# dohlee/diffab-pytorch

Measured on AMD Instinct MI355X. Metric: CDR-residue denoise-steps/sec (K=128 patch), higher is better.
Workload: dtype f32 (bf16x6 / fp16x3 split-precision products on the 16-bit matrix cores, fp32 accumulate; fp32-accurate, DESIGN section 4)

## Files before the change

### diffab-pytorch_amd/csrc/api.hip

```cpp
#include <atomic>
#include <cstring>
#include <mutex>
#include <vector>

#include "common.h"
#include "denoiser_internal.h"
#include "mlp_chain_tile.h"
#include "../../include/diffab_hip_debug.h"

namespace diffab {

static thread_local char g_err[512] = "";

void set_error(const char* fmt, ...) {
  va_list ap;
  va_start(ap, fmt);
  vsnprintf(g_err, sizeof(g_err), fmt, ap);
  va_end(ap);
}

namespace {
struct OrderState {
  std::recursive_mutex mu;
  hipStream_t last = nullptr;
// ... 362 lines not shown
  int* row_plan;
  unsigned char* start_class;
  float* beta_traj;
  int* ctx_of_row;
  float* res_ctx;
  void* step;
  size_t bytes;
};

static SampleBuffers carve_sample(const diffab_dims* d, void* ws, int n_pair = 0, bool mapped = false) {
  Carver c(ws);
  const size_t rows = static_cast<size_t>(d->B) * d->K;
  SampleBuffers s;
  s.beta = c.take<float>(d->B);
  s.eps = c.take<float>(rows * 3);
  s.O0 = c.take<float>(rows * 9);
  s.post = c.take<float>(rows * d->V);
  s.t_dev = c.take<int>(64);
  s.tiles = c.take<unsigned char>(static_cast<size_t>(d->B) * ((d->K + 15) / 16));
  s.row_plan = c.take<int>(static_cast<size_t>(d->B) * (2 + (d->K + 15) / 16));
  s.beta_traj = c.take<float>(static_cast<size_t>(3) * kTrajRows * d->D);
  s.ctx_of_row = mapped ? c.take<int>(d->B) : nullptr;
  s.res_ctx = mapped ? c.take<float>(rows * d->D) : nullptr;
  const size_t step_bytes = carve_step(d, nullptr, n_pair).bytes;
  s.step = c.take<char>(step_bytes);
  s.start_class = c.take<unsigned char>((static_cast<size_t>(d->B) + 3) & ~static_cast<size_t>(3));
  s.bytes = c.bytes();
  return s;
}

struct ScoreBuffers {
  int* t_list;
  float* beta;
  int* ctx_of_row;
  int64_t* seq_t;
  float *x_t, *O_t, *eps, *eps_hat;
  float* res_ctx;
  void* step;
  size_t bytes;
};
static ScoreBuffers carve_score(const diffab_dims* d, void* ws, int n_ctx) {
  Carver c(ws);
  const size_t rows = static_cast<size_t>(d->B) * d->K;
  ScoreBuffers s;
  s.t_list = c.take<int>(kTrajRows);
  s.beta = c.take<float>(d->B);
  s.ctx_of_row = c.take<int>(d->B);
  s.seq_t = c.take<int64_t>(rows);
  s.x_t = c.take<float>(rows * 3);
  s.O_t = c.take<float>(rows * 9);
  s.eps = c.take<float>(rows * 3);
  s.eps_hat = c.take<float>(rows * 3);
  s.res_ctx = c.take<float>(rows * d->D);
  s.step = c.take<char>(carve_step(d, nullptr, n_ctx).bytes);
  s.bytes = c.bytes();
  return s;
}

}

using namespace diffab;

extern "C" {

const char* diffab_version(void) { return "diffab_hip 0.1.0 (gfx950)"; }
const char* diffab_last_error(void) { return g_err; }

int diffab_device_ok(void) {
  int n = 0;
  if (hipGetDeviceCount(&n) != hipSuccess || n <= 0) return 0;
  hipDeviceProp_t p;
  int dev = 0;
  if (hipGetDevice(&dev) != hipSuccess || hipGetDeviceProperties(&p, dev) != hipSuccess) return 0;
  return std::strncmp(p.gcnArchName, "gfx950", 6) == 0 ? 1 : 0;
}

int diffab_debug_linear128(const float* X, const float* W, const float* bias, float* Y, int64_t M, int32_t Kd, int32_t mode, void* scratch,
                           size_t scratch_bytes, void* stream) {
  StreamOrder order_(stream);
  DIFFAB_REQUIRE(X && W && Y && M >= 1 && M < (1LL << 31) && Kd >= 32 && Kd % 32 == 0, DIFFAB_ERR_ARG, "debug_linear128: bad operands");
  hipStream_t st = as_stream(stream);
  if (mode == 0) return launch_linear(X, Kd, W, bias, Y, 128, static_cast<int>(M), 128, Kd, false, st);
  if (int rc = require_aligned16("debug_linear128", {{"X", X}, {"W", W}, {"bias", bias}, {"Y", Y}})) return rc;
  if (mode == 2) {
    const size_t pb = (rowgemm128_h3_planes_bytes(Kd) + 255) & ~static_cast<size_t>(255);
    DIFFAB_REQUIRE(Kd % 64 == 0, DIFFAB_ERR_ARG, "debug_linear128: mode 2 (fp16 x 3) needs Kd %% 64 == 0 (its chunks of 32 k are joined in pairs)");
    DIFFAB_REQUIRE(scratch && scratch_bytes >= pb + 512 && rowgemm128_b6_ok(X, Kd, Y, 128, static_cast<int>(M), Kd) &&
                       (reinterpret_cast<uintptr_t>(scratch) & 15) == 0,
                   DIFFAB_ERR_ARG, "debug_linear128: mode 2 needs 16-byte aligned operands and %zu bytes of scratch", pb + 512);
    float* wis = reinterpret_cast<float*>(static_cast<char*>(scratch) + pb);
    if (int rc = launch_wsplit128_h3(W, Kd, Kd, scratch, wis, st)) return rc;
    return launch_rowgemm128_h3p(X, Kd, scratch, wis, bias, nullptr, 0, Y, 128, static_cast<int>(M), Kd, false, st, nullptr);
  }
  DIFFAB_REQUIRE(mode == 1 && scratch && scratch_bytes >= rowgemm128_b6_scratch_bytes(Kd) && rowgemm128_b6_ok(X, Kd, Y, 128, static_cast<int>(M), Kd),
                 DIFFAB_ERR_ARG, "debug_linear128: mode 1 needs 16-byte aligned operands and %zu bytes of scratch", rowgemm128_b6_scratch_bytes(Kd));
  return launch_rowgemm128_b6(X, Kd, W, Kd, bias, nullptr, 0, Y, 128, static_cast<int>(M), Kd, false, scratch, st);
}

int diffab_debug_xstat128(const float* X, const float* W, float* Y, int64_t M, int32_t N, int32_t mode, void* scratch, size_t scratch_bytes,
                          void* stream) {
  StreamOrder order_(stream);
  DIFFAB_REQUIRE(X && W && Y && scratch && M >= 1 && M < (1LL << 31) && N >= 1 && (mode == 1 || mode == 2), DIFFAB_ERR_ARG,
                 "debug_xstat128: bad operands");
  const size_t need = mode == 1 ? xstat_b6_scratch_bytes(N) : xstat_h3_scratch_bytes(N);
  if (int rc = require_aligned16("debug_xstat128", {{"X", X}, {"W", W}, {"Y", Y}})) return rc;
  DIFFAB_REQUIRE(scratch_bytes >= need && (reinterpret_cast<uintptr_t>(scratch) & 15) == 0 && (reinterpret_cast<uintptr_t>(X) & 15) == 0,
                 DIFFAB_ERR_ARG, "debug_xstat128: needs 16-byte aligned X / scratch and %zu bytes of scratch", need);
  hipStream_t st = as_stream(stream);
  if (mode == 1) return launch_xstat_b6(X, W, 1, N, Y, N, static_cast<int>(M), N, scratch, st);
  return launch_xstat_h3(X, W, 1, N, Y, N, static_cast<int>(M), N, scratch, st);
}

int diffab_debug_dense_forms(int64_t rows, int32_t nblocks, int32_t has_parts, int32_t* out5) {
  DIFFAB_REQUIRE(out5 && rows >= 1 && rows < (1LL << 31) && nblocks >= 1, DIFFAB_ERR_ARG, "debug_dense_forms: bad operands");
  const int M = static_cast<int>(rows);
  const int group = rowgemm128_rows_per_group(M, has_parts != 0);
  out5[0] = group;
  out5[1] = M % (group == 0 ? 64 : group) != 0;
  out5[2] = dense_tile_full(M);
  out5[3] = dense_tile_nsplit(M, nblocks);
  out5[4] = M - (M - 1) / kDenseTileRows * kDenseTileRows;
  return DIFFAB_OK;
}

int diffab_debug_gemm_tn(const float* A, const float* B, float* C, float* db, int64_t M, int32_t N1, int32_t N2, int32_t mode, void* stream) {
  StreamOrder order_(stream);
  DIFFAB_REQUIRE(A && B && C && M >= 1 && M < (1LL << 31) && N1 >= 1 && N2 >= 1 && (mode == 1 || mode == 2), DIFFAB_ERR_ARG,
                 "debug_gemm_tn: bad operands");
  hipStream_t st = as_stream(stream);
  if (mode == 1) return launch_gemm_tn_b6(A, N1, B, N2, C, N2, static_cast<int>(M), N1, N2, db, nullptr, nullptr, 0, st);
  return launch_gemm_tn_h3(A, N1, B, N2, C, N2, static_cast<int>(M), N1, N2, db, nullptr, nullptr, 0, st);
}

int diffab_set_stream_guard(int on) {
  set_stream_order(on != 0);
  return DIFFAB_OK;
}

int diffab_debug_set_module_stagger(int32_t ticks_10ns, int32_t classes) {
  set_module_stagger(ticks_10ns, classes);
  return DIFFAB_OK;
}

int diffab_debug_set_module_stamps(void* device_buffer) {
  set_module_stamps(device_buffer);
  return DIFFAB_OK;
}

int diffab_debug_row_tiles(const uint8_t* gen_mask, int32_t B, int32_t K, uint8_t* tiles, void* stream) {
  StreamOrder order_(stream);
  DIFFAB_REQUIRE(gen_mask && tiles && B >= 1 && K >= 16 && K % 16 == 0, DIFFAB_ERR_ARG, "debug_row_tiles: need B >= 1 and K a multiple of 16");
  return launch_tiles_needed(gen_mask, B, K, tiles, as_stream(stream));
}

int diffab_debug_row_plan(const uint8_t* gen_mask, int32_t B, int32_t K, int32_t* plan, void* stream) {
  StreamOrder order_(stream);
  DIFFAB_REQUIRE(gen_mask && plan && B >= 1 && K >= 16 && K <= 1024 && K % 16 == 0, DIFFAB_ERR_ARG,
                 "debug_row_plan: need B >= 1 and K a multiple of 16 in 16 .. 1024");
  return launch_row_plan(gen_mask, B, K, plan, as_stream(stream));
}

int diffab_debug_start_classes(const int32_t* plan, int32_t B, int32_t K, int32_t classes, uint8_t* out, int32_t on_device, void* stream) {
  DIFFAB_REQUIRE(plan && out && B >= 1 && K >= 16 && K <= 1024 && K % 16 == 0 && classes >= 1 && classes <= 256, DIFFAB_ERR_ARG,
                 "debug_start_classes: need B >= 1, K a multiple of 16 in 16 .. 1024 and 1 .. 256 classes");
  if (on_device) {
    StreamOrder order_(stream);
    return launch_start_classes(plan, B, K, classes, out, as_stream(stream));
  }
  for (int b = 0; b < B; ++b) out[b] = static_cast<uint8_t>(start_class_of(plan, B, K, classes, b));
  return DIFFAB_OK;
}

int diffab_debug_set_attn_variant(int32_t v) { return set_attn_variant(v); }

// ... 674 lines not shown
```

### diffab-pytorch_amd/csrc/denoiser_internal.h

```cpp
#pragma once
#include "common.h"

namespace diffab {

int launch_linear_generic(const float* X, int ldx, const float* W, const float* bias, float* Y, int ldy, int M, int N, int Kd, bool relu,
                          hipStream_t st);
size_t ipa_generic_workspace_floats(const diffab_dims* d);
int ipa_layer_generic(const diffab_dims* d, const diffab_ipa_layer_weights* w, const float* x, const float* e, const float* R, const float* t,
                      float* y, float* ws, hipStream_t st, const int* ctx_of_row = nullptr);
int launch_embed_concat(const float* res_ctx, const float* emb, const int64_t* seq, int D, int64_t rows, float* out, hipStream_t st);
int launch_beta_concat(const float* h, const float* beta, int D, int K, int64_t rows, float* out, hipStream_t st);
int launch_heads_finish(const float* v, const float* O_t, const float* logits, int V, int64_t rows, float* O0, float* post, hipStream_t st);
int launch_proj_frames_f32(const float* x, const float* const* W6, const float* R, const float* t, float* proj, int rows, hipStream_t st);
int launch_losses_bwd(const float* post, const float* tpost, const float* eps, const float* teps, const float* O0, const float* tO,
                      const float* O_t, const float* v, const uint8_t* gm, const uint8_t* rm, const float* count, const float* up, int V,
                      int64_t rows, float* d_logits, float* d_eps, float* d_v, hipStream_t st);
int launch_heads_cotangent(const float* post, const float* c_post, const float* c_eps, const float* c_O0, const float* O_t, const float* v,
                           int V, int64_t rows, float* d_logits, float* d_eps, float* d_v, float* d_Ot, hipStream_t st);
int launch_ipa_frames_bwd(const float* proj, const float* dproj, int NP, int pt_col0, int n_pts, const float* feat, const float* dfeat, int F,
                          int ol_col0, int on_col0, int n_vpts, const float* R, const float* t, float* dR, float* dt, int rows,
                          hipStream_t st);

constexpr int kDenseTileRows = 128;
constexpr int kDenseFillGroups = 256;
constexpr int kPartsTilesMax = 64;
inline int rowgemm128_rows_per_group(int M, bool parts_usable) {
  if (parts_usable && (M + 63) / 64 <= kPartsTilesMax) return 0;
  return (M + kDenseTileRows - 1) / kDenseTileRows >= kDenseFillGroups ? 128 : 64;
}
inline bool dense_tile_full(int rows) { return rows % kDenseTileRows == 0; }
inline int dense_tile_nsplit(int rows, int nblocks) {
  const int ntiles = (rows + kDenseTileRows - 1) / kDenseTileRows, nsplit = kDenseFillGroups / ntiles;
  return nsplit < 1 ? 1 : (nsplit > nblocks ? nblocks : nsplit);
}

bool fast_path_supported(const diffab_dims* d);
size_t ipa_fast_workspace_floats(const diffab_dims* d);
int ipa_layer_fast(const diffab_dims* d, const diffab_ipa_layer_weights* w, const float* x, const float* e, const float* R, const float* t,
                   float* y, float* ws, hipStream_t st,
                   float* sp_keep = nullptr, float* d2_keep = nullptr,
                   const void* planes = nullptr,
                   const float* pair_planes = nullptr,
                   bool fp32_gemm = false,
                   bool taped = false,
                   const unsigned char* tile_needed = nullptr,
                   const int* ctx_of_row = nullptr, int n_ctx = 0);
bool pair_planes_supported(const diffab_dims* d);
size_t pair_planes_floats(const diffab_dims* d, int n_pair = 0);
int launch_pair_split(const diffab_dims* d, const float* e, float* planes, hipStream_t st, int n_pair = 0);
const float* pair_row_scales(const diffab_dims* d, const float* planes, int n_pair = 0);
int launch_linear(const float* X, int ldx, const float* W, const float* bias, float* Y, int ldy, int M, int N, int Kd, bool relu,
                  hipStream_t st);

bool rowgemm128_ok(const float* X, int ldx, const float* Y, int ldy, int M, int Kd);
int launch_rowgemm128(const float* X, int ldx, const float* W, int ldw, const float* bias, const int64_t* bias_idx, int bias_div, float* Y,
                      int ldy, int M, int Kd, bool relu, hipStream_t st);
size_t rowgemm128_b6_scratch_bytes(int Kd);
bool rowgemm128_b6_ok(const float* X, int ldx, const float* Y, int ldy, int M, int Kd);
int launch_wsplit128(const float* W, int ldw, int Kd, void* planes, hipStream_t st, int nrows = 128);
int launch_mlp_chains_b6(const float* X, int ldx, int nchains, const void* const* planes, const float* const* bias, const int64_t* bias_idx0,
                         int bias_div0, int nlayers, const int* n_out, float* const* Y, const int* ldy, int M, hipStream_t st);
struct MlpChainSet;
int make_mlp_chain_set(MlpChainSet* out, int nchains, const void* const* planes, const float* const* bias, const int64_t* bias_idx0,
                       int bias_div0, int nlayers, const int* n_out, float* const* Y, const int* ldy);
int launch_mlp_chain_b6(const float* X, int ldx, const void* const* planes, const float* const* bias, const int64_t* bias_idx0, int bias_div0,
                        int nlayers, int n_out, float* Y, int ldy, int M, hipStream_t st);
int launch_wsplit128_strided(const float* W, int64_t sn, int64_t sk, int kseg, int k0, void* planes, hipStream_t st);
int launch_wsplit128_segs(const float* const* W, const int* k_end, int nseg, void* planes, hipStream_t st);
int launch_rowgemm128_b6p(const float* X, int ldx, const void* planes, const float* bias, const int64_t* bias_idx, int bias_div, float* Y,
                          int ldy, int M, int Kd, bool relu, hipStream_t st, float* parts = nullptr);
size_t rowgemm128_b6_parts_floats(int M, int Kd);
size_t rowgemm128_h3_parts_floats(int M, int Kd);
int launch_rowgemm128_b6(const float* X, int ldx, const float* W, int ldw, const float* bias, const int64_t* bias_idx, int bias_div, float* Y,
                         int ldy, int M, int Kd, bool relu, void* scratch, hipStream_t st);
bool use_b6_gemm(uint32_t flags = 0);
size_t xstat_b6_scratch_bytes(int N);
int launch_gemm_tn_h3(const float* A, int lda, const float* B, int ldb, float* C, int ldc, int M, int N1, int N2, float* db,
                      float* const* seg_ptrs, const int* seg_ends, int nseg, hipStream_t st);
size_t xstat_h3_scratch_bytes(int N);
int launch_xstat_h3(const float* X, const float* W, int64_t sn, int64_t sk, float* Y, int ldy, int rows, int N, void* scratch, hipStream_t st);
int launch_xstat_b6(const float* X, const float* W, int64_t sn, int64_t sk, float* Y, int ldy, int rows, int N, void* scratch, hipStream_t st);
bool gemm_tn_b6_ok(const float* A, int lda, const float* B, int ldb, int M, int N1, int N2);
int launch_gemm_tn_b6(const float* A, int lda, const float* B, int ldb, float* C, int ldc, int M, int N1, int N2, float* db,
                      float* const* seg_ptrs, const int* seg_ends, int nseg, hipStream_t st);
size_t ipa_layer_planes_bytes();
size_t ipa_layer_small_offset();
size_t ipa_layer_h3_pj_offset();
size_t ipa_layer_h3_out_offset();
size_t ipa_layer_h3_wis_offset();
size_t rowgemm128_h3_planes_bytes(int Kd);
size_t proj_frames_h3_planes_bytes();
int launch_wsplit128_h3(const float* W, int ldw, int Kd, void* planes, float* wis, hipStream_t st, int nrows = 128);
int launch_pjsplit_h3(const float* const* W6, void* planes, float* wis, hipStream_t st);
int launch_rowgemm128_h3p(const float* X, int ldx, const void* planes, const float* wis, const float* bias, const int64_t* bias_idx, int bias_div,
                          float* Y, int ldy, int M, int Kd, bool relu, hipStream_t st, float* parts = nullptr);
int launch_proj_frames_h3p(const float* x, const void* planes, const float* wis, const float* R, const float* t, float* proj, int rows,
                           hipStream_t st);
int ipa_layer_split_weights(const diffab_ipa_layer_weights* w, void* planes, hipStream_t st);
bool ipa_module_persistent_supported(const diffab_dims* d);
int launch_ipa_module_persistent(const diffab_dims* d, float* xa, float* xb, const float* R, const float* t, float* ws, const void* planes,
                                 const float* pair_planes, hipStream_t st, const float* emb_X = nullptr, const MlpChainSet* emb = nullptr,
                                 const MlpChainSet* heads = nullptr, const int* ctx_of_row = nullptr, int n_ctx = 0,
                                 const int* last_layer_rows = nullptr,
                                 const unsigned char* start_class = nullptr);
int module_stagger_classes();
void set_module_stagger(int ticks, int classes);
void set_module_stamps(void* device_buffer);
int launch_fold_embed_table(const diffab_dims* d, const diffab_denoiser_weights* w, float* emb_tab, hipStream_t st);
int launch_fold_beta_table(const diffab_dims* d, const diffab_denoiser_weights* w, const float* beta, float* beta_tab, hipStream_t st,
                           const float* sched_beta = nullptr, int t = 0, const int* t_dev = nullptr);

bool pair_embed_fused_supported(const diffab_ctx_dims* d);
size_t pair_embed_fused_prep_floats(const diffab_ctx_dims* d);
int launch_pair_embed_fused(const diffab_ctx_dims* d, const diffab_pair_emb_weights* w, const int64_t* seq_idx, const float* distmat,
                            const float* xyz, const float* pairwise_dihedrals, const int64_t* residue_idx, int32_t residue_idx_batch_stride,
                            const int64_t* chain_idx, const float* atom_mask, const uint8_t* sequence_context_mask, float* out, float* prep,
                            float* tape_h1, float* tape_df, float* tape_m1, float* tape_m2, int64_t row0, int64_t nrows, hipStream_t st,
                            const float** coef_sp_out = nullptr);
int launch_softplus_table(const float* coefw, int n, float* out, hipStream_t st);

bool attention_split_supported(const diffab_dims* d);
size_t attention_split_workspace_floats(const diffab_dims* d);
int launch_ipa_logits(const diffab_dims* d, const float* proj, const float* gamma, float* SP, hipStream_t st);
int launch_attention_probs(const diffab_dims* d, const float* proj, const float* e, const float* Wb, const float* gamma, float* P,
                           float* D2, hipStream_t st);
constexpr int kDeLayersMax = 6;
int launch_pair_de_layers(const diffab_dims* d, int nl, const float* const* P, const float* const* G, const float* const* doe,
                          const float* const* Wb, float* de, hipStream_t st);
int launch_pair_stream_bwd(const diffab_dims* d, const float* e, const float* P, float* G , const float* D2,
                           const float* dfeat, float* wb_part, const float* Wb, float* de ,
                           hipStream_t st);
int launch_attention_split(const diffab_dims* d, const float* proj, const float* e, const float* R, const float* t, const float* Wb,
                           const float* gamma, float* feat, float* SP, hipStream_t st, float* D2 = nullptr);

void set_stream_order(bool on);
int set_attn_variant(int v);
void set_attn_stamps(void* device_buffer);

void timer_begin(hipStream_t st);
void timer_end(hipStream_t st);
bool kernel_timer_enabled();

struct Geometry {
  int rows, NP, F;
  size_t HKK;
  explicit Geometry(const diffab_dims* d)
      : rows(d->B * d->K), NP(3 * d->H * d->DS + 2 * d->H * d->PQ * 3 + d->H * d->PV * 3),
        F(d->H * d->DS + d->H * d->C + d->H * d->PV * 3 + d->H * d->PV), HKK(static_cast<size_t>(d->B) * d->H * d->K * d->K) {}
  size_t per_row(size_t n) const { return static_cast<size_t>(rows) * n; }
};

constexpr int kMaxLayers = 16;
struct BackwardPlan {
  bool fast;
  bool probs_on_tape;
  bool de_slots;
  bool split_planes;
};
BackwardPlan plan_backward(const diffab_dims* d);
struct TrainTape {
  float *cat2, *h1, *x[kMaxLayers + 1], *ipa_ws[kMaxLayers], *cat3, *t1[3], *t2[3], *vbuf, *logits;
  float* scratch;
  void* planes;
  float *sp[kMaxLayers], *d2[kMaxLayers];
  size_t floats;
};
TrainTape carve_tape(const diffab_dims* d, float* base);
inline size_t train_tape_floats(const diffab_dims* d) { return carve_tape(d, nullptr).floats; }
constexpr size_t kAttnBwdLdsMax = 160 * 1024;
size_t attn_bwd_lds_bytes(const diffab_dims* d);
inline bool attn_bwd_lds_ok(const diffab_dims* d) { return attn_bwd_lds_bytes(d) <= kAttnBwdLdsMax; }
size_t train_bwd_workspace_floats(const diffab_dims* d);
enum BwdRoot { BWD_LOSSES, BWD_COTANGENTS, BWD_LAYER };
struct BackwardArgs {
  BwdRoot root;
  const diffab_dims* d;
  const diffab_denoiser_weights *w, *g;
  TrainTape tp;
  float* ws;
  hipStream_t st;
  const int64_t* seq_t;
  const float *trans, *rot, *pair_ctx;
  const float *eps_hat, *O0_hat, *true_post, *true_eps, *true_O0, *upstream3;
  const uint8_t *gm, *rm;
  const float* post_hat;
  const float *cot_eps, *cot_O0, *cot_post;
  const float* layer_dy;
  float *layer_dx, *d_res_ctx, *d_pair_ctx, *d_trans, *d_rot;
};
int run_backward(const BackwardArgs& a);
// ... 145 lines not shown
```

### diffab-pytorch_amd/csrc/gemm_f16x3.hip

```cpp
#include "common.h"
#include "denoiser_internal.h"
#include "proj_frames_h3_tile.h"
#include "rowgemm_h3_tile.h"

namespace diffab {

using h3tile::BK;
using h3tile::h3_scale;
using h3tile::split2;

__global__ __launch_bounds__(256) void wsplit128_h3_kernel(const float* __restrict__ W, int ldw, int Kd, _Float16* __restrict__ out,
                                                          float* __restrict__ wis, int nrows) {
  const int n = blockIdx.x, tid = threadIdx.x;
  const float* row = W + static_cast<int64_t>(n) * ldw;
  float m = 0.0f;
  if (n < nrows)
    for (int k = tid; k < Kd; k += 256) m = fmaxf(m, fabsf(row[k]));
#pragma unroll
  for (int o = 1; o < 64; o <<= 1) m = fmaxf(m, __shfl_xor(m, o));
  __shared__ float wm[4];
  if ((tid & 63) == 0) wm[tid >> 6] = m;
  __syncthreads();
  m = fmaxf(fmaxf(wm[0], wm[1]), fmaxf(wm[2], wm[3]));
  float s, is;
  h3_scale(m, s, is);
  if (tid == 0) wis[n] = is;
  for (int k = tid; k < Kd; k += 256) {
    _Float16 h1, h2;
    split2(n < nrows ? row[k] * s : 0.0f, h1, h2);
    const int chunk = k / BK, kk = k % BK;
    const size_t base = (static_cast<size_t>(chunk) * 2 * 128 + n) * BK + kk;
    out[base] = h1;
    out[base + 128 * BK] = h2;
  }
}

template <bool RELU, int ROWS>
__global__ __launch_bounds__(ROWS * 4) void rowgemm128_h3_kernel(const float* __restrict__ X, int ldx, const _Float16* __restrict__ Wc,
                                                                 const float* __restrict__ wis, const float* __restrict__ bias,
                                                                 const int64_t* __restrict__ bias_idx, int bias_div, float* __restrict__ Y,
                                                                 int ldy, int M, int Kd) {
  extern __shared__ __attribute__((aligned(16))) _Float16 h3_lds[];
  h3tile::rowgemm128_h3_tile<RELU, ROWS>(h3_lds, threadIdx.x, blockIdx.x, X, ldx, Wc, wis, bias, bias_idx, bias_div, Y, ldy, M, Kd);
}
template <int ROWS>
__global__ __launch_bounds__(ROWS * 4) void rowgemm128_h3_parts_kernel(const float* __restrict__ X, int ldx, const _Float16* __restrict__ Wc, int M,
                                                                       int Kd, float* __restrict__ parts) {
  extern __shared__ __attribute__((aligned(16))) _Float16 h3_lds[];
  float* mine = parts + (static_cast<size_t>(blockIdx.x) * gridDim.y + blockIdx.y) * (ROWS * 128);
  h3tile::rowgemm128_h3_tile<false, ROWS, true>(h3_lds, threadIdx.x, blockIdx.x, X, ldx, Wc, nullptr, nullptr, nullptr, 0, nullptr, 0, M, Kd,
                                                blockIdx.y * h3tile::PART_CHUNKS, mine);
}
template <bool RELU, int ROWS>
__global__ __launch_bounds__(256) void rowgemm128_h3_parts_sum_kernel(const float* __restrict__ parts, int nparts, const float* __restrict__ wis,
                                                                      const float* __restrict__ bias, const int64_t* __restrict__ bias_idx,
                                                                      int bias_div, float* __restrict__ Y, int ldy, int M) {
  const int gid = blockIdx.x * 256 + threadIdx.x;
  const int row = gid >> 5, col = (gid & 31) * 4;
  if (row >= M) return;
  const float* src = parts + (static_cast<size_t>(row / ROWS) * nparts * ROWS + row % ROWS) * 128 + col;
  h3tile::f32x4 tot = {0.f, 0.f, 0.f, 0.f};
  for (int p = 0; p < nparts; ++p) {
    const h3tile::f32x4 v = *reinterpret_cast<const h3tile::f32x4*>(src + static_cast<size_t>(p) * (ROWS * 128));
#pragma unroll
    for (int c = 0; c < 4; ++c) tot[c] += v[c];
  }
  const bool table = bias_idx != nullptr || bias_div > 0;
  const float* brow = table ? bias + (bias_idx ? bias_idx[row] : row / bias_div) * 128 : bias;
#pragma unroll
  for (int c = 0; c < 4; ++c) {
    float o = __builtin_fmaf(tot[c], wis[col + c], brow ? brow[col + c] : 0.f);
    if (RELU) o = fmaxf(o, 0.f);
    Y[static_cast<int64_t>(row) * ldy + col + c] = o;
  }
}

size_t rowgemm128_h3_planes_bytes(int Kd) { return static_cast<size_t>(2) * 128 * Kd * sizeof(_Float16); }
bool rowgemm128_h3_ok(const float* X, int ldx, const float* Y, int ldy, int M, int Kd) {
  return Kd % BK == 0 && Kd >= BK && ldx % 4 == 0 && ldy % 4 == 0 && (reinterpret_cast<uintptr_t>(X) & 15) == 0 &&
         (reinterpret_cast<uintptr_t>(Y) & 15) == 0 && M >= 1;
}
int launch_wsplit128_h3(const float* W, int ldw, int Kd, void* planes, float* wis, hipStream_t st, int nrows) {
  DIFFAB_REQUIRE(W && planes && wis && (reinterpret_cast<uintptr_t>(planes) & 15) == 0 && Kd % BK == 0 && nrows >= 1 && nrows <= 128, DIFFAB_ERR_ARG,
                 "wsplit128_h3: bad operands");
  hipLaunchKernelGGL(wsplit128_h3_kernel, dim3(128), dim3(256), 0, st, W, ldw, Kd, static_cast<_Float16*>(planes), wis, nrows);
  DIFFAB_LAUNCH_CHECK();
  return DIFFAB_OK;
}
size_t rowgemm128_h3_parts_floats(int M, int Kd) {
  const size_t tiles64 = static_cast<size_t>((M + 63) / 64);
  return tiles64 <= kPartsTilesMax ? tiles64 * ((Kd / BK + h3tile::PART_CHUNKS - 1) / h3tile::PART_CHUNKS) * 64 * 128 : 0;
}
int launch_rowgemm128_h3p(const float* X, int ldx, const void* planes, const float* wis, const float* bias, const int64_t* bias_idx, int bias_div,
                          float* Y, int ldy, int M, int Kd, bool relu, hipStream_t st, float* parts) {
  DIFFAB_REQUIRE(rowgemm128_h3_ok(X, ldx, Y, ldy, M, Kd) && planes && wis && (reinterpret_cast<uintptr_t>(planes) & 15) == 0, DIFFAB_ERR_ARG,
                 "rowgemm128_h3: unsupported operands");
  const _Float16* Wc = static_cast<const _Float16*>(planes);
  const int tiles64 = (M + 63) / 64, nparts = (Kd / BK + h3tile::PART_CHUNKS - 1) / h3tile::PART_CHUNKS;
  const int rows_wg = rowgemm128_rows_per_group(M, parts && nparts > 1 && (reinterpret_cast<uintptr_t>(parts) & 15) == 0);
  if (rows_wg == 0) {
    DIFFAB_HIP_CHECK(hipFuncSetAttribute(reinterpret_cast<const void*>(rowgemm128_h3_parts_kernel<64>), hipFuncAttributeMaxDynamicSharedMemorySize,
                                         h3tile::lds_bytes<64>()));
    hipLaunchKernelGGL((rowgemm128_h3_parts_kernel<64>), dim3(tiles64, nparts), dim3(256), h3tile::lds_bytes<64>(), st, X, ldx, Wc, M, Kd, parts);
    const dim3 sgrid((M * 32 + 255) / 256);
    if (relu) hipLaunchKernelGGL((rowgemm128_h3_parts_sum_kernel<true, 64>), sgrid, dim3(256), 0, st, parts, nparts, wis, bias, bias_idx, bias_div, Y, ldy, M);
    else hipLaunchKernelGGL((rowgemm128_h3_parts_sum_kernel<false, 64>), sgrid, dim3(256), 0, st, parts, nparts, wis, bias, bias_idx, bias_div, Y, ldy, M);
    DIFFAB_LAUNCH_CHECK();
    return DIFFAB_OK;
  }
#define H3_LAUNCH(RELU_, ROWS_)                                                                                                          \
  do {                                                                                                                                   \
    DIFFAB_HIP_CHECK(hipFuncSetAttribute(reinterpret_cast<const void*>(rowgemm128_h3_kernel<RELU_, ROWS_>),                               \
                                         hipFuncAttributeMaxDynamicSharedMemorySize, h3tile::lds_bytes<ROWS_>()));                      \
    hipLaunchKernelGGL((rowgemm128_h3_kernel<RELU_, ROWS_>), dim3((M + ROWS_ - 1) / ROWS_), dim3(ROWS_ * 4), h3tile::lds_bytes<ROWS_>(), st, \
                       X, ldx, Wc, wis, bias, bias_idx, bias_div, Y, ldy, M, Kd);                                                        \
  } while (0)
  if (rows_wg == 128) {
    if (relu) H3_LAUNCH(true, 128);
    else H3_LAUNCH(false, 128);
  } else {
    if (relu) H3_LAUNCH(true, 64);
    else H3_LAUNCH(false, 64);
  }
#undef H3_LAUNCH
  DIFFAB_LAUNCH_CHECK();
  return DIFFAB_OK;
}

__global__ __launch_bounds__(64) void pjsplit_h3_kernel(const float* __restrict__ W0, const float* __restrict__ W1, const float* __restrict__ W2,
                                                        const float* __restrict__ W3, const float* __restrict__ W4, const float* __restrict__ W5,
                                                        _Float16* __restrict__ out, float* __restrict__ wis) {
  using namespace pjh3;
  const int gc = blockIdx.x, lane = threadIdx.x;
  const float* Wp;
  int row;
  if (gc < PJ_GQ) {
    Wp = gc < 256 ? W0 : (gc < 512 ? W1 : W2);
    row = gc & 255;
  } else {
    Wp = gc < 960 ? W3 : (gc < 1152 ? W4 : W5);
    row = gc - (gc < 960 ? PJ_GQ : (gc < 1152 ? 960 : 1152));
  }
  const float v0 = Wp[row * 128 + lane], v1 = Wp[row * 128 + 64 + lane];
  float m = fmaxf(fabsf(v0), fabsf(v1));
#pragma unroll
  for (int o = 1; o < 64; o <<= 1) m = fmaxf(m, __shfl_xor(m, o));
  float s, is;
  h3_scale(m, s, is);
  if (lane == 0) wis[gc] = is;
  const int blk = gc / PJ_B, rem = gc % PJ_B, cwl = rem / 48, r48 = rem % 48, j = r48 / 3, tt = r48 % 3;
  const int lrow = 48 * cwl + 16 * tt + j;
#pragma unroll
  for (int kh = 0; kh < 2; ++kh) {
    _Float16 h1, h2;
    split2((kh == 0 ? v0 : v1) * s, h1, h2);
    const size_t base = (static_cast<size_t>(blk * 2 + kh) * 2 * PJ_B + lrow) * 64 + lane;
    out[base] = h1;
    out[base + PJ_B * 64] = h2;
  }
}

template <bool FULL, bool SPLIT>
__global__ __launch_bounds__(512) void xstat_h3_kernel(const float* __restrict__ X, const _Float16* __restrict__ Wc, const float* __restrict__ wis,
                                                       float* __restrict__ Y, int M, int NB, int N, int ldy) {
  extern __shared__ __attribute__((aligned(16))) _Float16 pj_lds[];
  pjh3::proj_frames_h3_tile<FULL, SPLIT, false>(pj_lds, threadIdx.x, blockIdx.x, blockIdx.y, gridDim.y, X, Wc, wis, nullptr, nullptr, Y, M, NB, N, ldy);
}
__global__ __launch_bounds__(64) void xsplit_h3_kernel(const float* __restrict__ W, int64_t sn, int64_t sk, int N, _Float16* __restrict__ out,
                                                       float* __restrict__ wis) {
  using namespace pjh3;
  const int gc = blockIdx.x, lane = threadIdx.x;
  float v0 = 0.0f, v1 = 0.0f;
  if (gc < N) {
    v0 = W[gc * sn + lane * sk];
    v1 = W[gc * sn + (64 + lane) * sk];
  }
  float m = fmaxf(fabsf(v0), fabsf(v1));
#pragma unroll
  for (int o = 1; o < 64; o <<= 1) m = fmaxf(m, __shfl_xor(m, o));
  float s, is;
  h3_scale(m, s, is);
  if (lane == 0) wis[gc] = is;
  const int blk = gc / PJ_B, rem = gc % PJ_B, cwl = rem / 48, r48 = rem % 48, j = r48 / 3, tt = r48 % 3;
  const int lrow = 48 * cwl + 16 * tt + j;
#pragma unroll
  for (int kh = 0; kh < 2; ++kh) {
    _Float16 h1, h2;
    split2((kh == 0 ? v0 : v1) * s, h1, h2);
    const size_t base = (static_cast<size_t>(blk * 2 + kh) * 2 * PJ_B + lrow) * 64 + lane;
    out[base] = h1;
    out[base + PJ_B * 64] = h2;
  }
}

template <bool FULL, bool SPLIT>
__global__ __launch_bounds__(512) void proj_frames_h3_kernel(const float* __restrict__ X, const _Float16* __restrict__ Wc, const float* __restrict__ wis,
                                                             const float* __restrict__ R, const float* __restrict__ t, float* __restrict__ Y, int M) {
  extern __shared__ __attribute__((aligned(16))) _Float16 pj_lds[];
  pjh3::proj_frames_h3_tile<FULL, SPLIT>(pj_lds, threadIdx.x, blockIdx.x, blockIdx.y, gridDim.y, X, Wc, wis, R, t, Y, M);
}

size_t proj_frames_h3_planes_bytes() { return static_cast<size_t>(2 * pjh3::PJ_NB) * pjh3::PJ_STAGE_ELEMS * sizeof(_Float16); }
int launch_pjsplit_h3(const float* const* W6, void* planes, float* wis, hipStream_t st) {
  DIFFAB_REQUIRE(planes && wis && (reinterpret_cast<uintptr_t>(planes) & 15) == 0, DIFFAB_ERR_ARG, "pjsplit_h3: bad operands");
  hipLaunchKernelGGL(pjsplit_h3_kernel, dim3(pjh3::PJ_NP), dim3(64), 0, st, W6[0], W6[1], W6[2], W6[3], W6[4], W6[5],
                     static_cast<_Float16*>(planes), wis);
  DIFFAB_LAUNCH_CHECK();
// ... 354 lines not shown
```

### diffab-pytorch_amd/csrc/ipa_persistent.hip

```cpp
#include "common.h"
#include "denoiser_internal.h"
#define AT_STAMP_REALTIME 1
#include "ipa_attn_tile.h"
#include "proj_frames_h3_tile.h"
#include "rowgemm_h3_tile.h"
#include "mlp_chain_tile.h"
#include "mlp_chain_slab.h"

namespace diffab {

namespace {
constexpr size_t cmax(size_t a, size_t b) { return a > b ? a : b; }
constexpr size_t kModuleLdsBytes = cmax(cmax(ipa_attn_lds_bytes(8), static_cast<size_t>(kChainLdsBytes)),
                                        cmax(static_cast<size_t>(pjh3::PJ_LDS_BYTES), static_cast<size_t>(h3tile::lds_bytes<128>())));
constexpr size_t kXImageOffset = cmax(static_cast<size_t>(pjh3::PJ_LDS_BYTES), static_cast<size_t>(h3tile::lds_bytes<128>())) / 4;
static_assert(kXImageOffset * 4 + h3tile::y_lds_bytes<128>() <= kModuleLdsBytes, "module LDS: no room for the x image of the dense phases");
static_assert(kModuleLdsBytes <= 160 * 1024, "module LDS: one work-group per CU within gfx950's 160 KiB");
static_assert(kXImageOffset % 4 == 0, "x image: 16-byte aligned rows");

struct ModuleArgs {
  float* xa;
  float* xb;
  float* proj;
  float* feat;
  const float* pair;
  const float* esc;
  const int* ctx_of_row;
  const int* last_layer_rows;
  const float* R;
  const float* t;
  const char* planes;
  size_t layer_stride, pj_off, out_off, wis_off, small_off;
  unsigned long long* stamps;
  const float* emb_X;
  MlpChainSet emb, heads;
  int B, NL;
  int stagger_ticks, stagger_classes;
  const unsigned char* start_class;
};
}

__device__ __forceinline__ int module_plan_word(const int* __restrict__ plan, const int idx) {
  int w;
  asm volatile("s_load_dword %0, %1, 0x0\n\ts_waitcnt lgkmcnt(0)" : "=s"(w) : "s"(plan + idx) : "memory");
  return w;
}

template <int KRES, bool PLANNED_START = false>
__global__ __launch_bounds__(512) void ipa_module_persistent_kernel(const ModuleArgs a) {
  extern __shared__ __attribute__((aligned(16))) float lds[];
  constexpr int K = KRES, NTILE = K / TI, DT = K / 128;
  static_assert(KRES == 128 || KRES == 256, "patch-resident module: K = 128 or 256");
  const int M = a.B * K;
  if (a.stagger_ticks > 0 && a.stagger_classes > 1) {
    const unsigned long long t0 = __builtin_amdgcn_s_memrealtime();
    const int cls = PLANNED_START
                        ? (module_plan_word(reinterpret_cast<const int*>(a.start_class), blockIdx.x >> 2) >> (8 * (blockIdx.x & 3))) & 255
                        : static_cast<int>((blockIdx.x >> 3) % a.stagger_classes);
    const unsigned long long wait = static_cast<unsigned long long>(cls) * a.stagger_ticks;
    while (__builtin_amdgcn_s_memrealtime() - t0 < wait) __builtin_amdgcn_s_sleep(32);
  }
  unsigned long long* pstamps = a.stamps ? a.stamps + static_cast<size_t>(a.B) * a.NL * NTILE * 64 : nullptr;
  auto pstamp = [&](int b, int l, int k) {
    if (pstamps != nullptr && threadIdx.x == 0) pstamps[(static_cast<size_t>(b) * a.NL + l) * 4 + k] = __builtin_amdgcn_s_memrealtime();
  };
#pragma unroll 1
  for (int b = blockIdx.x; b < a.B; b += gridDim.x) {
    if (pstamps != nullptr && threadIdx.x == 0) pstamps[static_cast<size_t>(a.B) * a.NL * 4 + a.B + b] = __builtin_amdgcn_s_memrealtime();
    if (a.emb_X != nullptr) {
#pragma unroll 1
      for (int dt = 0; dt < DT; ++dt) {
        int tid = threadIdx.x;
        asm volatile("" : "+v"(tid));
        chaintile::mlp_chain_tile(reinterpret_cast<__bf16*>(lds), tid, b * DT + dt, a.emb_X, 128, a.emb.c[0].planes[0], a.emb.c[0].planes[1],
                                  nullptr, a.emb.c[0].bias[0], a.emb.c[0].bias[1], nullptr, a.emb.c[0].bias_idx0, a.emb.c[0].bias_div0, 2, 128,
                                  a.xa, 128, M);
        asm volatile("s_waitcnt vmcnt(0)" ::: "memory");
        __syncthreads();
      }
    }
#pragma unroll 1
    for (int l = 0; l < a.NL; ++l) {
      const char* lp = a.planes + static_cast<size_t>(l) * a.layer_stride;
      const float* small = reinterpret_cast<const float*>(lp + a.small_off);
      const float* xin = (l & 1) ? a.xb : a.xa;
      float* xout = (l & 1) ? a.xa : a.xb;
      pstamp(b, l, 0);
#pragma unroll 1
      for (int dt = 0; dt < DT; ++dt) {
        int tid = threadIdx.x;
        asm volatile("" : "+v"(tid));
        if (KRES == 128) {
          if (l == 0) {
            float* xl = lds + kXImageOffset;
            for (int i = tid; i < 128 * 32; i += 512) {
              const int row = i >> 5, c4 = 4 * (i & 31);
              *reinterpret_cast<float4*>(xl + row * h3tile::Y_LDS_LD + c4) =
                  *reinterpret_cast<const float4*>(xin + (static_cast<int64_t>(b) * 128 + row) * 128 + c4);
            }
            __syncthreads();
          }
          pjh3::proj_frames_h3_tile<true, false, true, true>(reinterpret_cast<_Float16*>(lds), tid, b, 0, 1, nullptr,
                                                             reinterpret_cast<const _Float16*>(lp + a.pj_off),
                                                             reinterpret_cast<const float*>(lp + a.wis_off), a.R, a.t, a.proj, M, 0, 0, 0,
                                                             lds + kXImageOffset);
        } else {
          pjh3::proj_frames_h3_tile<true, false>(reinterpret_cast<_Float16*>(lds), tid, b * DT + dt, 0, 1, xin,
                                                 reinterpret_cast<const _Float16*>(lp + a.pj_off), reinterpret_cast<const float*>(lp + a.wis_off),
                                                 a.R, a.t, a.proj, M);
        }
        if (dt + 1 < DT) {
          asm volatile("s_waitcnt vmcnt(0)" ::: "memory");
          __syncthreads();
        }
      }
      asm volatile("s_waitcnt vmcnt(0)" ::: "memory");
      __syncthreads();
      pstamp(b, l, 1);
      const int* rows = l + 1 == a.NL ? a.last_layer_rows : nullptr;
      const int n_items = rows != nullptr ? module_plan_word(rows, b * (2 + NTILE)) : NTILE;
#pragma unroll 1
      for (int item = 0; item < n_items; ++item) {
        const int i0 = rows != nullptr ? module_plan_word(rows, b * (2 + NTILE) + 2 + item) : item * TI;
        ipa_attn_tile<8, (KRES > 128), true>(lds, b, i0, static_cast<unsigned>((b * a.NL + l) * NTILE + item), a.proj, a.pair, a.R, a.t, small,
                                             small + 512, a.feat, K / 128, a.stamps, a.esc, nullptr, nullptr, a.ctx_of_row);
        asm volatile("s_waitcnt vmcnt(0)" ::: "memory");
        __syncthreads();
      }
      pstamp(b, l, 2);
#pragma unroll 1
      for (int dt = 0; dt < DT; ++dt) {
        int tid = threadIdx.x;
        asm volatile("" : "+v"(tid));
        if (KRES == 128)
          h3tile::rowgemm128_h3_tile<false, 128, false, true>(reinterpret_cast<_Float16*>(lds), tid, b, a.feat, AF,
                                                              reinterpret_cast<const _Float16*>(lp + a.out_off),
                                                              reinterpret_cast<const float*>(lp + a.wis_off) + ANP, small + 576, nullptr, 0,
                                                              l + 1 == a.NL ? xout : nullptr, 128, M, AF, 0, nullptr, lds + kXImageOffset);
        else
          h3tile::rowgemm128_h3_tile<false, 128>(reinterpret_cast<_Float16*>(lds), tid, b * DT + dt, a.feat, AF,
                                                 reinterpret_cast<const _Float16*>(lp + a.out_off),
                                                 reinterpret_cast<const float*>(lp + a.wis_off) + ANP, small + 576, nullptr, 0, xout, 128, M, AF);
        if (dt + 1 < DT) {
          asm volatile("s_waitcnt vmcnt(0)" ::: "memory");
          __syncthreads();
        }
      }
      asm volatile("s_waitcnt vmcnt(0)" ::: "memory");
      __syncthreads();
      pstamp(b, l, 3);
    }
    if (a.emb_X != nullptr) {
      const float* xfin = (a.NL & 1) ? a.xb : a.xa;
      if (KRES == 128 && a.last_layer_rows != nullptr) {
        unsigned rest = static_cast<unsigned>(module_plan_word(a.last_layer_rows, b * (2 + NTILE) + 1)) & 15u;
#pragma unroll 1
        while (rest != 0) {
          const int s0 = __builtin_ctz(rest);
          rest &= rest - 1;
          const int ns = rest != 0 ? 2 : 1;
          const int s1 = rest != 0 ? __builtin_ctz(rest) : s0;
          rest &= rest - 1;
          int tid = threadIdx.x;
          asm volatile("" : "+v"(tid));
          chainslab::mlp_chain_slabs<3>(reinterpret_cast<__bf16*>(lds), tid, ns, b * 128 + 32 * s0, b * 128 + 32 * s1, xfin, 128, a.heads, M);
        }
        asm volatile("s_waitcnt vmcnt(0)" ::: "memory");
      } else {
#pragma unroll 1
      for (int hdt = 0; hdt < 3 * DT; ++hdt) {
        const int hd = hdt / DT, dt = hdt % DT;
        const unsigned hslabs =
            a.last_layer_rows != nullptr ? static_cast<unsigned>(module_plan_word(a.last_layer_rows, b * (2 + NTILE) + 1)) : ~0u;
        const unsigned tslabs = (hslabs >> (4 * dt)) & 15u;
        if (tslabs == 0) continue;
        int tid = threadIdx.x;
        asm volatile("" : "+v"(tid));
#define HSEL(f) (hd == 0 ? a.heads.c[0].f : hd == 1 ? a.heads.c[1].f : a.heads.c[2].f)
        chaintile::mlp_chain_tile<true>(reinterpret_cast<__bf16*>(lds), tid, b * DT + dt, xfin, 128, HSEL(planes[0]), HSEL(planes[1]), HSEL(planes[2]),
                                  HSEL(bias[0]), HSEL(bias[1]), HSEL(bias[2]), HSEL(bias_idx0), HSEL(bias_div0), 3, HSEL(n_out),
                                  hd == 0 ? a.heads.Y[0] : hd == 1 ? a.heads.Y[1] : a.heads.Y[2],
                                  hd == 0 ? a.heads.ldy[0] : hd == 1 ? a.heads.ldy[1] : a.heads.ldy[2], M, tslabs);
#undef HSEL
        asm volatile("s_waitcnt vmcnt(0)" ::: "memory");
        __syncthreads();
      }
      }
      if (pstamps != nullptr && threadIdx.x == 0) pstamps[static_cast<size_t>(a.B) * a.NL * 4 + b] = __builtin_amdgcn_s_memrealtime();
    }
  }
}

namespace {
int g_stagger_ticks = 1000, g_stagger_classes = 8;
unsigned long long* g_module_stamps = nullptr;
}
void set_module_stagger(int ticks, int classes) {
  g_stagger_ticks = ticks;
  g_stagger_classes = classes;
}
void set_module_stamps(void* p) { g_module_stamps = static_cast<unsigned long long*>(p); }
int module_stagger_classes() { return g_stagger_ticks > 0 ? g_stagger_classes : 1; }

bool ipa_module_persistent_supported(const diffab_dims* d) {
  return fast_path_supported(d) && (d->K == 128 || d->K == 256) && d->NL >= 1;
}

int launch_ipa_module_persistent(const diffab_dims* d, float* xa, float* xb, const float* R, const float* t, float* ws, const void* planes,
                                 const float* pair_planes, hipStream_t st, const float* emb_X, const MlpChainSet* emb,
                                 const MlpChainSet* heads, const int* ctx_of_row, int n_ctx, const int* last_layer_rows,
                                 const unsigned char* start_class) {
  DIFFAB_REQUIRE(ipa_module_persistent_supported(d) && xa && xb && R && t && ws && planes && pair_planes, DIFFAB_ERR_ARG,
                 "ipa_module_persistent: unsupported operands");
  DIFFAB_REQUIRE((reinterpret_cast<uintptr_t>(last_layer_rows) & 3) == 0, DIFFAB_ERR_ARG,
                 "ipa_module_persistent: the row plan must be 4-byte aligned");
  const size_t rows = static_cast<size_t>(d->B) * d->K;
  ModuleArgs a{};
  a.xa = xa;
  a.xb = xb;
  a.proj = ws;
  a.feat = ws + rows * ANP;
  a.pair = pair_planes + 64;
  a.esc = pair_row_scales(d, pair_planes, n_ctx);
  a.ctx_of_row = ctx_of_row;
  a.last_layer_rows = last_layer_rows;
  a.R = R;
  a.t = t;
  a.planes = static_cast<const char*>(planes);
  a.layer_stride = ipa_layer_planes_bytes();
// ... 42 lines not shown
```

Baseline: 15.59 million.

## Compute attention output projection only on needed 32-row slabs in the last layer

Adds a slab-form fp16x3 row GEMM that computes the 128-wide output projection for only one or two 32-row slabs. In the persistent IPA module's last layer, when the plan marks at most two slabs as needed, this replaces the full 128-row tile loop. The goal is to skip MFMA work and X staging for rows whose output is never consumed. A debug entry point is also added for testing. It brings a new pipelined kernel with its own LDS layout and adds a branch to the persistent kernel, which may raise register pressure.

```diff
diff --git a/diffab-pytorch_amd/csrc/api.hip b/diffab-pytorch_amd/csrc/api.hip
--- a/diffab-pytorch_amd/csrc/api.hip
+++ b/diffab-pytorch_amd/csrc/api.hip
@@ -468,6 +468,8 @@
   hipStream_t st = as_stream(stream);
   if (mode == 0) return launch_linear(X, Kd, W, bias, Y, 128, static_cast<int>(M), 128, Kd, false, st);
   if (int rc = require_aligned16("debug_linear128", {{"X", X}, {"W", W}, {"bias", bias}, {"Y", Y}})) return rc;
+  const int slab_form = (mode & 255) == 3, slab0 = (mode >> 8) & 4095, slab1 = ((mode >> 20) & 4095) - 1;
+  if (slab_form) mode = 2;
   if (mode == 2) {
     const size_t pb = (rowgemm128_h3_planes_bytes(Kd) + 255) & ~static_cast<size_t>(255);
     DIFFAB_REQUIRE(Kd % 64 == 0, DIFFAB_ERR_ARG, "debug_linear128: mode 2 (fp16 x 3) needs Kd %% 64 == 0 (its chunks of 32 k are joined in pairs)");
@@ -476,6 +478,7 @@
                    DIFFAB_ERR_ARG, "debug_linear128: mode 2 needs 16-byte aligned operands and %zu bytes of scratch", pb + 512);
     float* wis = reinterpret_cast<float*>(static_cast<char*>(scratch) + pb);
     if (int rc = launch_wsplit128_h3(W, Kd, Kd, scratch, wis, st)) return rc;
+    if (slab_form) return launch_rowgemm128_h3_slabs(X, Kd, scratch, wis, bias, Y, 128, static_cast<int>(M), Kd, slab0, slab1, st);
     return launch_rowgemm128_h3p(X, Kd, scratch, wis, bias, nullptr, 0, Y, 128, static_cast<int>(M), Kd, false, st, nullptr);
   }
   DIFFAB_REQUIRE(mode == 1 && scratch && scratch_bytes >= rowgemm128_b6_scratch_bytes(Kd) && rowgemm128_b6_ok(X, Kd, Y, 128, static_cast<int>(M), Kd),
diff --git a/diffab-pytorch_amd/csrc/denoiser_internal.h b/diffab-pytorch_amd/csrc/denoiser_internal.h
--- a/diffab-pytorch_amd/csrc/denoiser_internal.h
+++ b/diffab-pytorch_amd/csrc/denoiser_internal.h
@@ -106,6 +106,8 @@
 int module_stagger_classes();
 void set_module_stagger(int ticks, int classes);
 void set_module_stamps(void* device_buffer);
+int launch_rowgemm128_h3_slabs(const float* X, int ldx, const void* planes, const float* wis, const float* bias, float* Y, int ldy, int M, int Kd,
+                               int slab0, int slab1, hipStream_t st);
 int launch_fold_embed_table(const diffab_dims* d, const diffab_denoiser_weights* w, float* emb_tab, hipStream_t st);
 int launch_fold_beta_table(const diffab_dims* d, const diffab_denoiser_weights* w, const float* beta, float* beta_tab, hipStream_t st,
                            const float* sched_beta = nullptr, int t = 0, const int* t_dev = nullptr);
diff --git a/diffab-pytorch_amd/csrc/gemm_f16x3.hip b/diffab-pytorch_amd/csrc/gemm_f16x3.hip
--- a/diffab-pytorch_amd/csrc/gemm_f16x3.hip
+++ b/diffab-pytorch_amd/csrc/gemm_f16x3.hip
@@ -2,6 +2,7 @@
 #include "denoiser_internal.h"
 #include "proj_frames_h3_tile.h"
 #include "rowgemm_h3_tile.h"
+#include "rowgemm_h3_slab.h"
 
 namespace diffab {
 
@@ -123,6 +124,35 @@
     else H3_LAUNCH(false, 64);
   }
 #undef H3_LAUNCH
+  DIFFAB_LAUNCH_CHECK();
+  return DIFFAB_OK;
+}
+
+template <int NS>
+__global__ __launch_bounds__(512) void rowgemm128_h3_slabs_kernel(const float* __restrict__ X, int ldx, const _Float16* __restrict__ Wc,
+                                                                  const float* __restrict__ wis, const float* __restrict__ bias,
+                                                                  float* __restrict__ Y, int ldy, int M, int Kd, int row0a, int row0b) {
+  extern __shared__ __attribute__((aligned(16))) _Float16 h3_lds[];
+  h3slab::rowgemm128_h3_slabs<NS>(h3_lds, threadIdx.x, row0a, row0b, X, ldx, Wc, wis, bias, Y, ldy, M, Kd);
+}
+int launch_rowgemm128_h3_slabs(const float* X, int ldx, const void* planes, const float* wis, const float* bias, float* Y, int ldy, int M, int Kd,
+                               int slab0, int slab1, hipStream_t st) {
+  DIFFAB_REQUIRE(rowgemm128_h3_ok(X, ldx, Y, ldy, M, Kd) && planes && wis && (reinterpret_cast<uintptr_t>(planes) & 15) == 0 && Kd % 128 == 0,
+                 DIFFAB_ERR_ARG, "rowgemm128_h3_slabs: unsupported operands");
+  DIFFAB_REQUIRE(slab0 >= 0 && 32 * static_cast<int64_t>(slab0) < M && slab1 != slab0 && (slab1 < 0 || 32 * static_cast<int64_t>(slab1) < M),
+                 DIFFAB_ERR_ARG, "rowgemm128_h3_slabs: slabs %d, %d outside the %d rows", slab0, slab1, M);
+  const _Float16* Wc = static_cast<const _Float16*>(planes);
+  if (slab1 >= 0) {
+    DIFFAB_HIP_CHECK(hipFuncSetAttribute(reinterpret_cast<const void*>(rowgemm128_h3_slabs_kernel<2>), hipFuncAttributeMaxDynamicSharedMemorySize,
+                                         h3slab::lds_bytes()));
+    hipLaunchKernelGGL((rowgemm128_h3_slabs_kernel<2>), dim3(1), dim3(512), h3slab::lds_bytes(), st, X, ldx, Wc, wis, bias, Y, ldy, M, Kd,
+                       32 * slab0, 32 * slab1);
+  } else {
+    DIFFAB_HIP_CHECK(hipFuncSetAttribute(reinterpret_cast<const void*>(rowgemm128_h3_slabs_kernel<1>), hipFuncAttributeMaxDynamicSharedMemorySize,
+                                         h3slab::lds_bytes()));
+    hipLaunchKernelGGL((rowgemm128_h3_slabs_kernel<1>), dim3(1), dim3(512), h3slab::lds_bytes(), st, X, ldx, Wc, wis, bias, Y, ldy, M, Kd,
+                       32 * slab0, 0);
+  }
   DIFFAB_LAUNCH_CHECK();
   return DIFFAB_OK;
 }
diff --git a/diffab-pytorch_amd/csrc/ipa_persistent.hip b/diffab-pytorch_amd/csrc/ipa_persistent.hip
--- a/diffab-pytorch_amd/csrc/ipa_persistent.hip
+++ b/diffab-pytorch_amd/csrc/ipa_persistent.hip
@@ -4,6 +4,7 @@
 #include "ipa_attn_tile.h"
 #include "proj_frames_h3_tile.h"
 #include "rowgemm_h3_tile.h"
+#include "rowgemm_h3_slab.h"
 #include "mlp_chain_tile.h"
 #include "mlp_chain_slab.h"
 
@@ -128,6 +129,25 @@
         __syncthreads();
       }
       pstamp(b, l, 2);
+      unsigned oslabs = 0xffu;
+      if (PLANNED_START && rows != nullptr && a.emb_X != nullptr)
+        oslabs = static_cast<unsigned>(module_plan_word(rows, b * (2 + NTILE) + 1)) & 15u;
+      if (PLANNED_START && __builtin_popcount(oslabs) <= 2) {
+        if (oslabs != 0) {
+          const int s0 = __builtin_ctz(oslabs);
+          const unsigned rest = oslabs & (oslabs - 1);
+          int tid = threadIdx.x;
+          asm volatile("" : "+v"(tid));
+          const _Float16* wo = reinterpret_cast<const _Float16*>(lp + a.out_off);
+          const float* wos = reinterpret_cast<const float*>(lp + a.wis_off) + ANP;
+          if (rest != 0)
+            h3slab::rowgemm128_h3_slabs<2>(reinterpret_cast<_Float16*>(lds), tid, b * 128 + 32 * s0, b * 128 + 32 * __builtin_ctz(rest), a.feat,
+                                           AF, wo, wos, small + 576, xout, 128, M, AF);
+          else
+            h3slab::rowgemm128_h3_slabs<1>(reinterpret_cast<_Float16*>(lds), tid, b * 128 + 32 * s0, 0, a.feat, AF, wo, wos, small + 576, xout,
+                                           128, M, AF);
+        }
+      } else {
 #pragma unroll 1
       for (int dt = 0; dt < DT; ++dt) {
         int tid = threadIdx.x;
@@ -145,6 +165,7 @@
           asm volatile("s_waitcnt vmcnt(0)" ::: "memory");
           __syncthreads();
         }
+      }
       }
       asm volatile("s_waitcnt vmcnt(0)" ::: "memory");
       __syncthreads();
diff --git a/diffab-pytorch_amd/csrc/rowgemm_h3_slab.h b/diffab-pytorch_amd/csrc/rowgemm_h3_slab.h
--- /dev/null
+++ b/diffab-pytorch_amd/csrc/rowgemm_h3_slab.h
@@ -0,0 +1,164 @@
+#pragma once
+#include <hip/hip_runtime.h>
+#include <cstdint>
+
+#include "rowgemm_h3_tile.h"
+
+namespace diffab {
+namespace h3slab {
+using h3tile::BK;
+using h3tile::f16x4;
+using h3tile::f16x8;
+using h3tile::f32x16;
+using h3tile::f32x4;
+using h3tile::h3_off;
+using h3tile::h3_scale;
+using h3tile::split2;
+typedef const f16x8 __attribute__((address_space(1)))* global_f16x8_p;
+
+constexpr int PH_CHUNKS = 4;
+constexpr int kSlabImage = PH_CHUNKS * 2 * 32 * BK;
+constexpr int lds_bytes() { return 2 * 2 * kSlabImage * 2 + 2 * 2 * 2 * 32 * 4; }
+
+template <int NS>
+__device__ __forceinline__ void rowgemm128_h3_slabs(_Float16* sl, const int tid, const int row0a, const int row0b, const float* __restrict__ X,
+                                                    int ldx, const _Float16* __restrict__ Wc, const float* __restrict__ wis,
+                                                    const float* __restrict__ bias, float* __restrict__ Y, int ldy, int M, int Kd) {
+  static_assert(NS == 1 || NS == 2, "slab form: one slab or two");
+  float* Sx = reinterpret_cast<float*>(sl + 2 * 2 * kSlabImage);
+  const int lane = tid & 63, l31 = lane & 31, hk = lane >> 5;
+  const int wv_u = __builtin_amdgcn_readfirstlane(tid >> 6);
+  const bool has_unit = wv_u < 4;
+  const int cg = wv_u & 3;
+  const int nchunk = Kd / BK, nphase = nchunk / PH_CHUNKS;
+  const unsigned w_lane = static_cast<unsigned>(((32 * cg + l31) * BK + 8 * hk) * 2);
+  f16x8 wf[PH_CHUNKS][2][2];
+  auto load_w = [&](int slot, int ch) {
+    ch = ch < nchunk ? ch : nchunk - 1;
+    const _Float16* src = Wc + static_cast<size_t>(ch) * (2 * 128 * BK);
+#pragma unroll
+    for (int ks = 0; ks < 2; ++ks)
+#pragma unroll
+      for (int p = 0; p < 2; ++p)
+        wf[slot][ks][p] = *(global_f16x8_p)(reinterpret_cast<uintptr_t>(src + (p * 128) * BK + 16 * ks) + w_lane);
+  };
+  if (has_unit) {
+#pragma unroll
+    for (int c = 0; c < PH_CHUNKS; ++c) load_w(c, c);
+  }
+  const float* xsrc[NS][2];
+#pragma unroll
+  for (int j = 0; j < NS; ++j)
+#pragma unroll
+    for (int i = 0; i < 2; ++i) {
+      const int q = tid + 512 * i;
+      int row = (j ? row0b : row0a) + (q >> 5);
+      row = row < M ? row : M - 1;
+      xsrc[j][i] = X + static_cast<int64_t>(row) * ldx + 4 * (q & 31);
+    }
+  f32x4 xr[NS][2];
+  auto load_x = [&](int ph) {
+    ph = ph < nphase ? ph : nphase - 1;
+#pragma unroll
+    for (int j = 0; j < NS; ++j)
+#pragma unroll
+      for (int i = 0; i < 2; ++i) xr[j][i] = *reinterpret_cast<const f32x4*>(xsrc[j][i] + ph * (PH_CHUNKS * BK));
+  };
+  auto stage = [&](int buf) {
+#pragma unroll
+    for (int j = 0; j < NS; ++j)
+#pragma unroll
+      for (int i = 0; i < 2; ++i) {
+        const int q = tid + 512 * i, lrow = q >> 5, c4 = q & 31;
+        const f32x4 v = xr[j][i];
+        float m = fmaxf(fmaxf(fabsf(v[0]), fabsf(v[1])), fmaxf(fabsf(v[2]), fabsf(v[3])));
+        m = fmaxf(m, __shfl_xor(m, 1));
+        m = fmaxf(m, __shfl_xor(m, 2));
+        m = fmaxf(m, __shfl_xor(m, 4));
+        m = fmaxf(m, __shfl_xor(m, 8));
+        float s, is;
+        h3_scale(m, s, is);
+        if ((c4 & 15) == 0) Sx[((buf * 2 + j) * 2 + (c4 >> 4)) * 32 + lrow] = is;
+        f16x4 h1, h2;
+#pragma unroll
+        for (int c = 0; c < 4; ++c) {
+          _Float16 a, b;
+          split2(v[c] * s, a, b);
+          h1[c] = a; h2[c] = b;
+        }
+        _Float16* dst = sl + (buf * 2 + j) * kSlabImage + (c4 >> 3) * (2 * 32 * BK) + h3_off(lrow, (c4 & 7) >> 1) + 4 * (c4 & 1);
+        *reinterpret_cast<f16x4*>(dst) = h1;
+        *reinterpret_cast<f16x4*>(dst + 32 * BK) = h2;
+      }
+  };
+  f32x16 acc[NS], tot[NS];
+#pragma unroll
+  for (int j = 0; j < NS; ++j)
+#pragma unroll
+    for (int r = 0; r < 16; ++r) acc[j][r] = tot[j][r] = 0.f;
+  load_x(0);
+  stage(0);
+  __syncthreads();
+  const int fx = (l31 >> 2) & 3;
+#pragma unroll 1
+  for (int ph = 0; ph < nphase; ++ph) {
+    const int buf = ph & 1;
+    load_x(ph + 1);
+    if (has_unit) {
+      const _Float16* al = sl + (buf * 2) * kSlabImage + l31 * BK;
+#pragma unroll
+      for (int c = 0; c < PH_CHUNKS; ++c) {
+#pragma unroll
+        for (int ks = 0; ks < 2; ++ks) {
+          const int so = 8 * ((2 * ks + hk) ^ fx);
+          f16x8 a[NS][2];
+#pragma unroll
+          for (int j = 0; j < NS; ++j)
+#pragma unroll
+            for (int p = 0; p < 2; ++p) a[j][p] = *reinterpret_cast<const f16x8*>(al + j * kSlabImage + (c * 2 + p) * (32 * BK) + so);
+#pragma unroll
+          for (int j = 0; j < NS; ++j) acc[j] = __builtin_amdgcn_mfma_f32_32x32x16_f16(a[j][1], wf[c][ks][0], acc[j], 0, 0, 0);
+#pragma unroll
+          for (int j = 0; j < NS; ++j) acc[j] = __builtin_amdgcn_mfma_f32_32x32x16_f16(a[j][0], wf[c][ks][1], acc[j], 0, 0, 0);
+#pragma unroll
+          for (int j = 0; j < NS; ++j) acc[j] = __builtin_amdgcn_mfma_f32_32x32x16_f16(a[j][0], wf[c][ks][0], acc[j], 0, 0, 0);
+        }
+        load_w(c, PH_CHUNKS * (ph + 1) + c);
+        __builtin_amdgcn_sched_barrier(0);
+        if (c & 1) {
+#pragma unroll
+          for (int j = 0; j < NS; ++j) {
+            f32x4 sx[4];
+#pragma unroll
+            for (int g = 0; g < 4; ++g) sx[g] = *reinterpret_cast<const f32x4*>(Sx + ((buf * 2 + j) * 2 + (c >> 1)) * 32 + 8 * g + 4 * hk);
+#pragma unroll
+            for (int r = 0; r < 16; ++r) {
+              tot[j][r] = __builtin_fmaf(acc[j][r], sx[r >> 2][r & 3], tot[j][r]);
+              acc[j][r] = 0.f;
+            }
+          }
+        }
+      }
+    }
+    stage(buf ^ 1);
+    __syncthreads();
+  }
+  if (has_unit) {
+    const int col = 32 * cg + l31;
+    const float wi = wis[col];
+    const float bv = bias ? bias[col] : 0.0f;
+#pragma unroll
+    for (int j = 0; j < NS; ++j) {
+      int row0 = j ? row0b : row0a;
+      asm volatile("" : "+v"(row0));
+#pragma unroll
+      for (int r = 0; r < 16; ++r) {
+        const int row = row0 + (r & 3) + 8 * (r >> 2) + 4 * hk;
+        if (row >= M) continue;
+        Y[static_cast<int64_t>(row) * ldy + col] = __builtin_fmaf(tot[j][r], wi, bv);
+      }
+    }
+  }
+}
+}
+}
```

New measurement: 15.72 million (median of 6 runs). No clear change (+0.8%).
